# charlesq34/pointnet2

Measured on NVIDIA H100. Metric: set-abstraction points/sec, higher is better.
Workload: dtype f32

## Files before the change

include/pn2_api.h:

```cpp
#ifndef PN2_API_H_
#define PN2_API_H_

#include <stddef.h>

#ifdef __cplusplus
extern "C" {
#endif

#define PN2_API_VERSION 2


int pn2_fps(int b, int n, int m, const float* inp, float* temp, int* out, void* stream);

size_t pn2_fps_scratch_bytes(int b, int n);

int pn2_fps_gather(int b, int n, int m, const float* inp, float* temp, int* out, float* new_xyz, void* stream);


int pn2_fps_gather_ragged(int b, int n, int m, const float* inp, const int* lengths, float* temp, int* out,
                          float* new_xyz, void* stream);

int pn2_prob_sample(int b, int n, int m, const float* inp_p, const float* inp_r, float* temp, int* out, void* stream);

int pn2_gather_point(int b, int n, int m, const float* inp, const int* idx, float* out, void* stream);
// ... 184 lines not shown
size_t pn2_scene_blocks_workspace_bytes(int p, int nx, int ny);
int pn2_scene_blocks_count(int p, const float* xyz, double lo_x, double lo_y, double block_size, double stride, double padding,
                           int nx, int ny, int* counts, void* workspace, size_t workspace_bytes, void* stream);
int pn2_scene_blocks_fill(int p, const float* xyz, double lo_x, double lo_y, double block_size, double stride, double padding,
                          int nx, int ny, const int* sub_begin, const int* sub_count, int b, int n, float* out_xyz,
                          int* point_idx, unsigned char* core, int* occ_off, int* occ_row, void* workspace,
                          size_t workspace_bytes, void* stream);
int pn2_scene_merge_typed(int dtype, int p, int c, int b, int n, int row_begin, int row_end, const void* logits,
                          const int* point_idx, const unsigned char* core, const int* occ_off, const int* occ_row,
                          float* accum, void* stream);

size_t pn2_scene_crops_workspace_bytes(int b, int npoints);
int pn2_scene_crops(int s, int p, int max_scene, const float* xyz, const int* label, const long long* offsets, const float* lo,
                    const float* hi, int num_class, const float* label_weights, int b, const long long* crop_scene,
                    long long seed, const long long* seed_dev, int npoints, double max_dropout, int rotate, float* out_xyz,
                    long long* out_label, float* out_weight, int* lengths, int* point_idx, unsigned char* core, int* attempt,
                    unsigned char* valid, void* workspace, size_t workspace_bytes, void* stream);

int pn2_shape_batch(int s, int p, int max_shape, const float* xyz, const float* normals, const int* label, const int* part,
                    const long long* offsets, int b, const long long* shape_idx, long long seed, const long long* seed_dev,
                    int votes, int npoints, int subset_random, int rotate, int perturb, int scale_on, double scale_lo,
                    double scale_hi, double shift, int jitter_on, double jitter_sigma, double jitter_clip,
                    double max_dropout, int with_normals, float* out_points, long long* out_label, long long* out_part,
                    int* lengths, int* point_idx, void* stream);

size_t pn2_virtual_scans_workspace_bytes(int b, int max_scene, int npoints);
int pn2_virtual_scans(int s, int p, int max_scene, const float* xyz, const int* label, const long long* offsets,
                      const double* mean, int num_class, const float* label_weights, int b, const long long* scan_scene,
                      const long long* scan_mode, long long seed, const long long* seed_dev, int npoints, int min_points,
                      float* out_xyz, long long* out_label, float* out_weight, int* lengths, int* point_idx, int* visible,
                      unsigned char* valid, void* workspace, size_t workspace_bytes, void* stream);

size_t pn2_render_balls_workspace_bytes(int b, int h, int w);
int pn2_render_balls(int b, int n, int h, int w, const int* xyz, const float* colors, const int* lengths, int r,
                     const unsigned char* background, void* workspace, size_t workspace_bytes, unsigned char* out,
                     void* stream);
int pn2_render_balls_counted(int b, int n, int h, int w, const int* xyz, const float* colors, const int* lengths, int r,
                             const unsigned char* background, void* workspace, size_t workspace_bytes,
                             unsigned char* out, unsigned long long* counters, void* stream);
int pn2_project_points(int b, int n, int v, const double* xyz, const int* lengths, const double* rotations, int size,
                       void* workspace, size_t workspace_bytes, int* out, void* stream);


size_t pn2_sa_layer_workspace_bytes(int b, int n, int m, int nsample);
int pn2_sa_layer_host(int b, int n, int m, float radius, int nsample, const float* h_xyz,
                      float* h_new_xyz, int* h_idx, int* h_pts_cnt, float* h_grouped_xyz,
                      void* workspace, size_t workspace_bytes, void* stream);

int pn2_api_version(void);
const char* pn2_error_string(int code);
unsigned long long pn2_launch_count(void);
float pn2_ball_threshold(float radius);
void pn2_set_fps_config(int threads, int points_per_thread, int cluster);
int pn2_fps_plan(int b, int n, int* threads, int* points_per_thread, int* cluster);
int pn2_fps_cluster_capacity(int threads, int points_per_thread, int cluster);
void pn2_set_bq_group(int lanes_per_query);
void pn2_set_bq_mode(int mode);

#ifdef __cplusplus
}
#endif
#endif
```

pointnet2_b200/_lib.py:

```python
from __future__ import annotations

import ctypes
import os
from ctypes import c_double, c_float, c_int, c_longlong, c_size_t, c_ulonglong, c_void_p

from . import _build

_P = c_void_p
_SIGNATURES = {
    "pn2_fps": (c_int, [c_int, c_int, c_int, _P, _P, _P, _P]),
    "pn2_fps_scratch_bytes": (c_size_t, [c_int, c_int]),
    "pn2_fps_gather": (c_int, [c_int, c_int, c_int, _P, _P, _P, _P, _P]),
    "pn2_prob_sample": (c_int, [c_int, c_int, c_int, _P, _P, _P, _P, _P]),
    "pn2_gather_point": (c_int, [c_int, c_int, c_int, _P, _P, _P, _P]),
    "pn2_gather_point_grad": (c_int, [c_int, c_int, c_int, _P, _P, _P, _P]),
    "pn2_gather_point_grad_det": (c_int, [c_int, c_int, c_int, _P, _P, _P, _P, c_size_t, _P]),
    "pn2_query_ball_point": (c_int, [c_int, c_int, c_int, c_float, c_int, _P, _P, _P, _P, _P]),
    "pn2_query_ball_point_workspace_bytes": (c_size_t, [c_int, c_int]),
    "pn2_query_ball_point_ws": (c_int, [c_int, c_int, c_int, c_float, c_int, _P, _P, _P, _P, _P, c_size_t, _P]),
    "pn2_ball_grid_build": (c_int, [c_int, c_int, c_float, c_int, _P, _P, c_size_t, _P]),
    "pn2_query_ball_point_prebuilt": (c_int, [c_int, c_int, c_int, c_float, c_int, _P, _P, _P, _P, _P, c_size_t, _P]),
    "pn2_group_point": (c_int, [c_int, c_int, c_int, c_int, c_int, _P, _P, _P, _P]),
    "pn2_group_point_grad": (c_int, [c_int, c_int, c_int, c_int, c_int, _P, _P, _P, _P]),
    "pn2_group_point_grad_det_workspace_bytes": (c_size_t, [c_int, c_int, c_int, c_int]),
# ... 33 lines not shown
    "pn2_three_nn_ragged": (c_int, [c_int, c_int, c_int, _P, _P, _P, _P, _P, _P]),
    "pn2_three_nn_interpolate_ragged_typed": (c_int, [c_int, c_int, c_int, c_int, c_int, _P, _P, _P, _P, _P, _P, _P, _P, _P]),
    "pn2_fp_interpolate_concat_ragged_typed": (c_int, [c_int, c_int, c_int, c_int, c_int, c_int, _P, _P, _P, _P, _P, _P, _P]),
    "pn2_three_interpolate_ragged_typed": (c_int, [c_int, c_int, c_int, c_int, c_int, _P, _P, _P, _P, _P, _P]),
    "pn2_three_interpolate_grad_ragged": (c_int, [c_int, c_int, c_int, c_int, _P, _P, _P, _P, _P, _P]),
    "pn2_three_interpolate_grad_det_ragged_typed": (c_int, [c_int, c_int, c_int, c_int, c_int, _P, _P, _P, _P, _P, _P, c_size_t, _P]),
    "pn2_masked_bn_workspace_bytes": (c_size_t, [c_int, c_int]),
    "pn2_masked_bn_relu_forward_typed": (c_int, [c_int, c_int, c_int, _P, _P, _P, _P, c_float, c_float, _P, _P, _P, _P, _P, _P, _P,
                                                 c_size_t, _P]),
    "pn2_masked_bn_relu_backward_typed": (c_int, [c_int, c_int, c_int, _P, _P, _P, _P, _P, _P, _P, _P, _P, _P, _P, c_size_t, _P]),
    "pn2_masked_bn_relu_max_workspace_bytes": (c_size_t, [c_int, c_int, c_int]),
    "pn2_masked_bn_relu_max_forward_typed": (c_int, [c_int, c_int, c_int, c_int, _P, _P, _P, _P, c_float, c_float, _P, _P, _P,
                                                     _P, _P, _P, _P, _P, c_size_t, _P]),
    "pn2_masked_bn_relu_max_backward_typed": (c_int, [c_int, c_int, c_int, c_int, _P, _P, _P, _P, _P, _P, _P, _P, _P, _P, _P,
                                                      _P, c_size_t, _P]),
    "pn2_sa_mlp_max_typed": (c_int, [c_int, c_int, c_int, c_int, c_int, c_int, _P, _P, _P, _P, c_int, c_int, c_int, _P, _P, _P,
                                     _P, _P, _P, _P, _P, _P, _P, c_longlong, _P]),
    "pn2_sa_mlp_max_all_workspace_bytes": (c_size_t, [c_int, c_int]),
    "pn2_sa_mlp_max_all_typed": (c_int, [c_int, c_int, c_int, c_int, _P, _P, _P, _P, c_int, c_int, c_int, _P, _P, _P, _P, _P,
                                         _P, _P, _P, _P, _P, c_longlong, _P, c_size_t, _P]),
    "pn2_fp_mlp_workspace_bytes": (c_size_t, [c_int, c_int]),
    "pn2_fp_mlp_typed": (c_int, [c_int, c_int, c_int, c_int, c_int, c_int, _P, _P, _P, _P, _P, c_int, _P, _P, _P, _P, _P, _P,
                                 _P, _P, _P, _P, c_longlong, _P, c_size_t, _P]),
    "pn2_mlp_rows_typed": (c_int, [c_int, c_longlong, c_int, _P, _P, c_int, _P, _P, _P, _P, _P, _P, _P, _P, _P, _P, c_longlong,
                                   _P]),
    "pn2_scene_blocks_workspace_bytes": (c_size_t, [c_int, c_int, c_int]),
    "pn2_scene_blocks_count": (c_int, [c_int, _P, c_double, c_double, c_double, c_double, c_double, c_int, c_int, _P, _P,
                                       c_size_t, _P]),
    "pn2_scene_blocks_fill": (c_int, [c_int, _P, c_double, c_double, c_double, c_double, c_double, c_int, c_int, _P, _P,
                                      c_int, c_int, _P, _P, _P, _P, _P, _P, c_size_t, _P]),
    "pn2_scene_merge_typed": (c_int, [c_int, c_int, c_int, c_int, c_int, c_int, c_int, _P, _P, _P, _P, _P, _P, _P]),
    "pn2_scene_crops_workspace_bytes": (c_size_t, [c_int, c_int]),
    "pn2_scene_crops": (c_int, [c_int, c_int, c_int, _P, _P, _P, _P, _P, c_int, _P, c_int, _P, c_longlong, _P, c_int, c_double,
                                c_int, _P, _P, _P, _P, _P, _P, _P, _P, _P, c_size_t, _P]),
    "pn2_shape_batch": (c_int, [c_int, c_int, c_int, _P, _P, _P, _P, _P, c_int, _P, c_longlong, _P, c_int, c_int, c_int,
                                c_int, c_int, c_int, c_double, c_double, c_double, c_int, c_double, c_double, c_double,
                                c_int, _P, _P, _P, _P, _P, _P]),
    "pn2_virtual_scans_workspace_bytes": (c_size_t, [c_int, c_int, c_int]),
    "pn2_virtual_scans": (c_int, [c_int, c_int, c_int, _P, _P, _P, _P, c_int, _P, c_int, _P, _P, c_longlong, _P, c_int, c_int,
                                  _P, _P, _P, _P, _P, _P, _P, _P, c_size_t, _P]),
    "pn2_render_balls_workspace_bytes": (c_size_t, [c_int, c_int, c_int]),
    "pn2_render_balls": (c_int, [c_int, c_int, c_int, c_int, _P, _P, _P, c_int, _P, _P, c_size_t, _P, _P]),
    "pn2_render_balls_counted": (c_int, [c_int, c_int, c_int, c_int, _P, _P, _P, c_int, _P, _P, c_size_t, _P, _P, _P]),
    "pn2_project_points": (c_int, [c_int, c_int, c_int, _P, _P, _P, c_int, _P, c_size_t, _P, _P]),
    "pn2_sa_layer_workspace_bytes": (c_size_t, [c_int, c_int, c_int, c_int]),
    "pn2_sa_layer_host": (c_int, [c_int, c_int, c_int, c_float, c_int, _P, _P, _P, _P, _P, _P, c_size_t, _P]),
    "pn2_api_version": (c_int, []),
    "pn2_error_string": (ctypes.c_char_p, [c_int]),
    "pn2_launch_count": (c_ulonglong, []),
    "pn2_ball_threshold": (c_float, [c_float]),
    "pn2_fps_plan": (c_int, [c_int, c_int, _P, _P, _P]),
    "pn2_fps_cluster_capacity": (c_int, [c_int, c_int, c_int]),
    "pn2_set_fps_config": (None, [c_int, c_int, c_int]),
    "pn2_set_bq_group": (None, [c_int]),
    "pn2_set_bq_mode": (None, [c_int]),
}

EXPORTED_SYMBOLS = tuple(_SIGNATURES)

_lib = None


def lib_path() -> str:
    return _build.LIB_PATH


def load() -> ctypes.CDLL:
    global _lib
    if _lib is not None:
        return _lib
    path = _build.LIB_PATH
    world = int(os.environ.get("WORLD_SIZE", "1") or "1")
    local_rank = int(os.environ.get("LOCAL_RANK", "0") or "0")
    if world > 1:
        want = _build.source_signature()
        stamp = path + ".stamp"
        if local_rank == 0:
            if _build.is_stale():
                try:
                    _build.build()
                except Exception as e:
                    if not os.path.exists(path):
                        raise ImportError(f"libpn2_b200.so is missing and could not be built: {e}") from e
                    want = "prebuilt"
            tmp = stamp + f".tmp{os.getpid()}"
            with open(tmp, "w") as f:
                f.write(want)
            os.replace(tmp, stamp)
        else:
            import time
            deadline = time.time() + 600
            while time.time() < deadline:
                try:
                    got = open(stamp).read()
                except OSError:
                    got = None
                if got in (want, "prebuilt") and os.path.exists(path):
                    break
                time.sleep(0.2)
            else:
                raise ImportError("libpn2_b200.so was not (re)built by local rank 0 within 10 minutes")
    elif _build.is_stale():
        try:
            _build.build()
        except Exception as e:
            if not os.path.exists(path):
# ... 26 lines not shown
```

pointnet2_b200/csrc/fps.cu:

```cuda
#include <stdio.h>
#include <stdlib.h>

#include <atomic>
#include <mutex>

#include "pn2_common.cuh"

namespace pn2 {

__device__ __forceinline__ unsigned tb_encode(unsigned k) { return ((k & 511u) << 23) | (k >> 9); }
__device__ __forceinline__ unsigned tb_decode(unsigned tb) { return ((tb & 0x7fffffu) << 9) | (tb >> 23); }

__device__ __forceinline__ unsigned smem_addr(const void* p) { return (unsigned)__cvta_generic_to_shared(p); }
__device__ __forceinline__ unsigned cluster_ctarank() {
    unsigned r;
    asm volatile("mov.u32 %0, %%cluster_ctarank;" : "=r"(r));
    return r;
}
__device__ __forceinline__ unsigned cluster_nctarank() {
    unsigned r;
    asm volatile("mov.u32 %0, %%cluster_nctarank;" : "=r"(r));
    return r;
}
__device__ __forceinline__ void cluster_sync_all() {
// ... 214 lines not shown
        Z[h] = f2_pack(c[0][2], c[1][2]);
    }
    const unsigned tp = (tid < n) ? tb_encode((unsigned)tid) : 0xffffffffu;

    float x1 = src[0], y1 = src[1], z1 = src[2];
    if (tid == 0) write_pick(out, oxyz, 0, 0, x1, y1, z1);
    if (tid < 64) (&s_keys[0][0])[tid] = make_uint2(0xffffffffu, 0u);
    __syncthreads();

#pragma unroll 2
    for (int it = 1; it < m; ++it) {
        pair_update(X, Y, Z, td, x1, y1, z1);
        float g[G];
#pragma unroll
        for (int a = 0; a < G; ++a) {
            float v = td[GS * a];
#pragma unroll
            for (int u = 1; u < GS; ++u) v = fmaxf(v, td[GS * a + u]);
            g[a] = v;
        }
        float mx = 0.0f;
#pragma unroll
        for (int a = 0; a < G; ++a) mx = fmaxf(mx, g[a]);
        float s[GS];
#pragma unroll
        for (int u = 0; u < GS; ++u) s[u] = td[GS * (G - 1) + u];
        unsigned cg = SO::tbj(GS * (G - 1));
#pragma unroll
        for (int a = G - 2; a >= 0; --a) {
            const bool q = (g[a] == mx);
#pragma unroll
            for (int u = 0; u + 1 < GS; ++u) s[u] = q ? td[GS * a + u] : s[u];
            cg = q ? SO::tbj(GS * a) : cg;
        }
        unsigned cu = SO::tbj(GS - 1);
#pragma unroll
        for (int u = GS - 2; u >= 0; --u) cu = (s[u] == mx) ? SO::tbj(u) : cu;
        unsigned hi = __float_as_uint(mx), lo = tp | cg | cu;
        warp_max_min_pair(hi, lo);
        const int buf = it & 1;
        s_keys[buf][warp] = make_uint2(lo, hi);
        __syncthreads();
        const uint2 e = s_keys[buf][lane];
        unsigned gh = e.y, gl = e.x;
        warp_max_min_pair(gh, gl);
        const int old = (int)tb_decode(gl);
        x1 = src[3 * old + 0];
        y1 = src[3 * old + 1];
        z1 = src[3 * old + 2];
        if (tid == 0) write_pick(out, oxyz, it, old, x1, y1, z1);
    }
}

template <int P, int T, int V = 0, bool L = false>
__global__ void __launch_bounds__(T, 1)
fps_cta_kernel(int n, int m, const float* __restrict__ xyz, int* __restrict__ idx_out,
               float* __restrict__ new_xyz, int sentinel, const int* __restrict__ lengths) {
    static_assert(T % 512 == 0 || 512 % T == 0, "T must divide or be a multiple of the reference's 512 slots");
    __shared__ uint2 s_keys[2][32];
    extern __shared__ __align__(16) float s_xyz[];

    const int tid = threadIdx.x, lane = tid & 31, warp = tid >> 5;
    const int cloud = blockIdx.x;
    const float* __restrict__ pts = xyz + (size_t)cloud * n * 3;
    int* __restrict__ out = idx_out + (size_t)cloud * m;
    float* __restrict__ oxyz = new_xyz ? new_xyz + (size_t)cloud * m * 3 : nullptr;
    const int nb = L ? cloud_length(lengths, cloud, n) : n;

    const int total = 3 * nb;
    const bool vec = (reinterpret_cast<size_t>(pts) & 15) == 0;
    const int nv = vec ? (total >> 2) : 0;
    const float4* __restrict__ p4 = reinterpret_cast<const float4*>(pts);
    float4* __restrict__ s4 = reinterpret_cast<float4*>(s_xyz);
    constexpr int LB = 12;
    float4 v[LB];
#pragma unroll
    for (int u = 0; u < LB; ++u) {
        const int e = u * T + tid;
        if (e < nv) v[u] = __ldg(p4 + e);
    }
    if (sentinel) {
        for (int e = tid; e < m; e += T) out[e] = -1;
        __threadfence();
    }
#pragma unroll
    for (int u = 0; u < LB; ++u) {
        const int e = u * T + tid;
        if (e < nv) s4[e] = v[u];
    }
    for (int base = LB * T; base < nv; base += LB * T) {
#pragma unroll
        for (int u = 0; u < LB; ++u) {
            const int e = base + u * T + tid;
            if (e < nv) v[u] = __ldg(p4 + e);
        }
#pragma unroll
        for (int u = 0; u < LB; ++u) {
            const int e = base + u * T + tid;
            if (e < nv) s4[e] = v[u];
        }
    }
#pragma unroll 8
    for (int e = (nv << 2) + tid; e < total; e += T) s_xyz[e] = pts[e];
    __syncthreads();
    if (sentinel) pdl_launch_dependents();
    const float* __restrict__ src = s_xyz;

    if constexpr (V == 1) {
        fps_chain_packed<P, T>(nb, m, src, out, oxyz, s_keys);
    } else {
        constexpr int NW = T / 32;
        float px[P], py[P], pz[P], td[P];
#pragma unroll
        for (int j = 0; j < P; ++j) {
            const int k = tid + j * T;
            if (k < nb) {
                px[j] = src[3 * k + 0];
                py[j] = src[3 * k + 1];
                pz[j] = src[3 * k + 2];
                td[j] = 1e38f;
            } else {
                px[j] = py[j] = pz[j] = 0.0f;
                td[j] = -1.0f;
            }
        }

        float x1 = src[0], y1 = src[1], z1 = src[2];
        if (tid == 0) write_pick(out, oxyz, 0, 0, x1, y1, z1);

        for (int it = 1; it < m; ++it) {
            float best;
            int bj;
            fps_step<P, ScanOrder<P, T>::DD>(px, py, pz, td, x1, y1, z1, best, bj);
            unsigned hi = 0u, lo = 0u;
            if (best >= 0.0f) {
                hi = __float_as_uint(best);
                lo = ~tb_encode((unsigned)(tid + bj * T));
            }
            warp_max_pair(hi, lo);
            const int buf = it & 1;
            if (lane == 0) s_keys[buf][warp] = make_uint2(lo, hi);
            __syncthreads();
            uint2 e = (lane < NW) ? s_keys[buf][lane] : make_uint2(0u, 0u);
            unsigned gh = e.y, gl = e.x;
            warp_max_pair(gh, gl);
            const int old = (int)tb_decode(~gl);
            x1 = src[3 * old + 0];
            y1 = src[3 * old + 1];
            z1 = src[3 * old + 2];
            if (tid == 0) write_pick(out, oxyz, it, old, x1, y1, z1);
        }
    }
}

__device__ __forceinline__ void init_step_mbars(unsigned long long (&s_mbar)[2]) {
    mbar_init(smem_addr(&s_mbar[0]), 1);
    mbar_init(smem_addr(&s_mbar[1]), 1);
    fence_mbar_init_cluster();
}

template <int P, int PR, int T, class Keep>
// ... 368 lines not shown
                const float d2 = fminf(d, td[k]);
                td[k] = d2;
                if (d2 > best) {
                    best = d2;
                    bk = k;
                }
            }
            unsigned hi = 0u, lo = 0u;
            if (best >= 0.0f) {
                hi = __float_as_uint(best);
                lo = ~tb_encode((unsigned)bk);
            }
            warp_max_pair(hi, lo);
            const int buf = it & 1;
            if (lane == 0) s_keys[buf][warp] = make_uint2(lo, hi);
            __syncthreads();
            uint2 e = (lane < NW) ? s_keys[buf][lane] : make_uint2(0u, 0u);
            unsigned gh = e.y, gl = e.x;
            warp_max_pair(gh, gl);
            const int old = (int)tb_decode(~gl);
            x1 = pts[3 * (size_t)old + 0];
            y1 = pts[3 * (size_t)old + 1];
            z1 = pts[3 * (size_t)old + 2];
            if (tid == 0) {
                out[it] = old;
                if (oxyz) {
                    oxyz[3 * it + 0] = x1;
                    oxyz[3 * it + 1] = y1;
                    oxyz[3 * it + 2] = z1;
                }
            }
        }
        __syncthreads();
    }
}

static std::atomic<unsigned long long> g_fps_cfg{0ull};
static std::once_flag g_fps_env_once;
constexpr int kFpsPackedDefault = 1;
static std::atomic<int> g_fps_packed{kFpsPackedDefault};
constexpr int kFpsPackedClusterDefault = 1;
static std::atomic<int> g_fps_packed_cluster{kFpsPackedClusterDefault};

static int override_chain(int threads, int builtin) {
    const int chain = threads & 3;
    return chain == 1 ? 1 : (chain == 2 ? 0 : builtin);
}

static unsigned long long pack_cfg(int threads, int ppt, int cluster) {
    if (threads <= 0) return 0ull;
    return ((unsigned long long)threads << 40) | ((unsigned long long)(ppt & 0xfffff) << 20) | (unsigned long long)(cluster + 64);
}

template <int P, int T, int V>
static int launch_cta(int b, int n, int m, const float* inp, const int* lengths, int* out, float* new_xyz, int sentinel,
                      cudaStream_t st) {
    static AttrOnce once[2];
    auto kern = lengths ? fps_cta_kernel<P, T, V, true> : fps_cta_kernel<P, T, V, false>;
    size_t dyn = (size_t)n * 3 * sizeof(float);
    if (dyn > 200 * 1024) return (int)cudaErrorInvalidValue;
    constexpr size_t kExclusive = 116 * 1024;
    if (2 * b <= num_sms() && dyn < kExclusive) dyn = kExclusive;
    cudaError_t e = ensure_attrs(once[lengths ? 1 : 0], kern, 200 * 1024, false);
    if (e != cudaSuccess) return (int)e;
    kern<<<b, T, dyn, st>>>(n, m, inp, out, new_xyz, sentinel, lengths);
    return finish_launch();
}

static cudaLaunchConfig_t cluster_config(int clusters, int C, int T, size_t dyn, cudaStream_t st, cudaLaunchAttribute* attr) {
    cudaLaunchConfig_t cfg = {};
    cfg.gridDim = dim3((unsigned)clusters * (unsigned)C, 1, 1);
    cfg.blockDim = dim3(T, 1, 1);
    cfg.dynamicSmemBytes = dyn;
    cfg.stream = st;
    attr[0].id = cudaLaunchAttributeClusterDimension;
    attr[0].val.clusterDim.x = C;
    attr[0].val.clusterDim.y = 1;
    attr[0].val.clusterDim.z = 1;
    cfg.attrs = attr;
    cfg.numAttrs = 1;
    return cfg;
}

template <int P, int T, int PR, int V>
struct ClusterKernel {
    static constexpr size_t dyn = (size_t)3 * P * T * sizeof(float), max_dyn = 200 * 1024;
    static constexpr int threads = T;
    static auto kernel(bool ragged = false) { return ragged ? fps_cluster_kernel<P, T, PR, V, true> : fps_cluster_kernel<P, T, PR, V, false>; }
};
template <int P, int T, int PR, int V>
struct ClusterBigKernel {
    static constexpr size_t dyn = (size_t)3 * (P - PR) * T * sizeof(float), max_dyn = 226 * 1024;
    static constexpr int threads = T;
    static auto kernel(bool ragged = false) {
        return ragged ? fps_cluster_big_kernel<P, T, PR, V, true> : fps_cluster_big_kernel<P, T, PR, V, false>;
    }
};

template <class K>
static int launch_cluster(int C, int cluster_arg, int b, int n, int m, const float* inp, const int* lengths, int* out,
                          float* new_xyz, cudaStream_t st) {
    static AttrOnce once[2];
    if (K::dyn > K::max_dyn) return (int)cudaErrorInvalidValue;
    const bool ragged = lengths != nullptr;
    cudaError_t e = ensure_attrs(once[ragged ? 1 : 0], K::kernel(ragged), K::dyn, true);
    if (e != cudaSuccess) return (int)e;
    cudaLaunchAttribute attr[1];
    const cudaLaunchConfig_t cfg = cluster_config(b, C, K::threads, K::dyn, st, attr);
    e = cudaLaunchKernelEx(&cfg, K::kernel(ragged), n, m, cluster_arg, inp, out, new_xyz, lengths);
    count_launch();
    if (e != cudaSuccess) return (int)e;
    return (int)cudaGetLastError();
}

template <class K>
static int cluster_capacity(int C) {
    static std::atomic<int> cache[17][64];
    int dev = 0;
    if (C < 2 || C > 16 || cudaGetDevice(&dev) != cudaSuccess || dev < 0 || dev >= 64) return 0;
    const int hit = cache[C][dev].load(std::memory_order_relaxed);
    if (hit) return hit > 0 ? hit : 0;
    static AttrOnce once;
    if (K::dyn > K::max_dyn || ensure_attrs(once, K::kernel(), K::dyn, true) != cudaSuccess) return 0;
    cudaLaunchAttribute attr[1];
    const cudaLaunchConfig_t cfg = cluster_config(num_sms(), C, K::threads, K::dyn, nullptr, attr);
    int num = 0;
    if (cudaOccupancyMaxActiveClusters(&num, K::kernel(), &cfg) != cudaSuccess) {
        (void)cudaGetLastError();
        num = 0;
    }
    cache[C][dev].store(num > 0 ? num : -1, std::memory_order_relaxed);
    return num;
}

#define PN2_FPS_CTA_KERNELS(X)                                                                       \
    X(1, 128, 0) X(2, 128, 0) X(4, 128, 0) X(8, 128, 1) X(16, 128, 1) X(32, 128, 1)                  \
    X(1, 256, 0) X(2, 256, 0) X(4, 256, 0) X(8, 256, 1) X(16, 256, 1) X(32, 256, 1)                  \
    X(1, 512, 0) X(2, 512, 0) X(4, 512, 0) X(8, 512, 1) X(16, 512, 1)                                \
    X(1, 1024, 0) X(2, 1024, 0) X(4, 1024, 0) X(8, 1024, 1)
#define PN2_FPS_CLUSTER_KERNELS(X)                                                                   \
    X(4, 128, 4, 1) X(8, 128, 8, 1) X(16, 128, 16, 1) X(32, 128, 32, 1)                              \
    X(2, 256, 2, 0) X(4, 256, 4, 1) X(8, 256, 8, 1) X(16, 256, 16, 1) X(32, 256, 32, 1)              \
    X(1, 512, 1, 0) X(2, 512, 2, 0) X(4, 512, 4, 1) X(8, 512, 8, 1) X(16, 512, 16, 1) X(32, 512, 16, 1) \
    X(2, 1024, 2, 0) X(4, 1024, 4, 1) X(8, 1024, 8, 1)
#define PN2_FPS_BIG_KERNELS(X) X(44, 16) X(48, 12) X(52, 16)

struct FpsPlan {
    int threads, ppt, cluster;
    int pr;
    int packed = 0;
};

static int pow2_floor(int v) {
    int p = 1;
    while (p * 2 <= v) p *= 2;
    return p;
}

int fps_cluster_capacity(int threads, int ppt, int cluster, int packed);

static FpsPlan plan_fps(int b, int n) {
    std::call_once(g_fps_env_once, [] {
        const char* e = getenv("PN2_FPS_CFG");
        int t = 0, pp = 0, c = 0;
        if (e && sscanf(e, "%d,%d,%d", &t, &pp, &c) == 3) g_fps_cfg.store(pack_cfg(t, pp, c), std::memory_order_relaxed);
        const char* pk = getenv("PN2_FPS_PACKED");
        if (pk && (pk[0] == '0' || pk[0] == '1') && pk[1] == 0) g_fps_packed.store(pk[0] - '0', std::memory_order_relaxed);
        const char* pc = getenv("PN2_FPS_PACKED_CLUSTER");
        if (pc && (pc[0] == '0' || pc[0] == '1') && pc[1] == 0) g_fps_packed_cluster.store(pc[0] - '0', std::memory_order_relaxed);
    });
    const int packed = g_fps_packed.load(std::memory_order_relaxed);
    const int packed_cluster = g_fps_packed_cluster.load(std::memory_order_relaxed);
    const unsigned long long ov = g_fps_cfg.load(std::memory_order_relaxed);
    if (ov) {
        FpsPlan p;
        p.threads = (int)(ov >> 40);
        p.ppt = (int)((ov >> 20) & 0xfffff);
        p.cluster = (int)(ov & 0xfffff) - 64;
        p.packed = override_chain(p.threads, (p.cluster >= 2) ? packed_cluster : packed);
        p.threads &= ~3;
        p.pr = (p.ppt >= 32 && p.threads >= 512) ? 16 : p.ppt;
        if (p.cluster == -1 || p.cluster == -2) {
            p.packed = (p.cluster == -2) ? 1 : 0;
            p.cluster = 1;
        }
        return p;
    }
    if (n <= 128) return {128, 1, 1, 1, packed};
    if (n <= 256) return {128, 2, 1, 2, packed};
    if (n <= 512) return {256, 2, 1, 2, packed};
    if (n <= 1024) return {128, 8, 1, 8, packed};
    if (n <= 2048) return {128, 16, 1, 16, packed};
    if (n <= 4096) return {256, 16, 1, 16, packed};
    if (n <= 8192) return {256, 32, 1, 32, packed};
    const int sms = num_sms();
    int cmax = pow2_floor(sms / (b > sms ? sms : b));
    if (cmax > 16) cmax = 16;
    if (cmax < 2) cmax = 2;
    auto pick = [packed_cluster](long long per, int C, FpsPlan& out) -> bool {
        const int t = (C >= 4) ? 128 : 256;
        const int pmin = (t == 128) ? 4 : 2;
        for (int pp = pmin; pp <= 32; pp *= 2) {
            if (per <= (long long)t * pp) {
                out = {t, pp, C, pp, packed_cluster};
                return true;
            }
        }
        if (per <= 256LL * 32) {
            out = {256, 32, C, 32, packed_cluster};
            return true;
        }
        if (per <= 512LL * 32) {
            out = {512, 32, C, 16, packed_cluster};
            return true;
        }
        return false;
    };
    FpsPlan first{0, 0, 0, 0};
    for (int C = cmax; C >= 2; C /= 2) {
        const long long per = ((long long)n + C - 1) / C;
        if (per <= 1024 && C > 2) continue;
        FpsPlan p;
        if (!pick(per, C, p)) break;
        if (first.cluster == 0) first = p;
        const int cap = fps_cluster_capacity(p.threads, p.ppt, p.cluster, p.packed);
        if (cap == 0 || cap >= b) return p;
    }
    FpsPlan best{0, 0, 0, 0};
    double best_cost = 1e30;
    auto consider = [&](const FpsPlan& p) {
        const int cap = fps_cluster_capacity(p.threads, p.ppt, p.cluster, p.packed);
        const int waves = cap > 0 ? (b + cap - 1) / cap : 1;
        double cost = waves * (0.3 + 0.07e-3 * (double)p.threads * p.ppt);
        if (cap > 0 && (long long)cap * p.cluster > sms) cost *= 1.3;
        if (cost < best_cost) {
            best_cost = cost;
            best = p;
        }
    };
    if (first.cluster) consider(first);
    FpsPlan widest;
    if (pick(((long long)n + 15) / 16, 16, widest)) consider(widest);
    for (int C = 16; C >= 2; --C) {
        const long long per = ((long long)n + C - 1) / C;
        if (per > 512LL * 52) break;
        consider({512, per <= 512LL * 44 ? 44 : (per <= 512LL * 48 ? 48 : 52), C, 16, packed_cluster});
    }
    if (best.cluster) return best;
    return {1024, 0, 0, 0};
}

bool fps_single_cta(int b, int n) { return plan_fps(b, n).cluster == 1; }

size_t fps_scratch_bytes(int b, int n) {
    if (b <= 0 || n <= 0) return 0;
    return plan_fps(b, n).cluster == 0 ? sizeof(float) * (size_t)(b < 32 ? b : 32) * (size_t)n : 0;
}

int fps_dispatch(int b, int n, int m, const float* inp, const int* lengths, float* temp, int* out, float* new_xyz,
                 int sentinel, cudaStream_t st) {
    if (b < 0 || n <= 0 || m < 0) return (int)cudaErrorInvalidValue;
    if (b == 0 || m == 0) return 0;
    if (!inp || !out) return (int)cudaErrorInvalidValue;
    const FpsPlan plan = plan_fps(b, n);
    if (sentinel && plan.cluster != 1) return (int)cudaErrorInvalidValue;
    if (plan.cluster >= 1) {
        const long long cap = (long long)plan.threads * plan.ppt * plan.cluster;
        if (cap < n) return (int)cudaErrorInvalidValue;
    }
    if (plan.cluster == 1) {
#define PN2_TRY(P, T, PK)                                                                           \
    if (plan.ppt == P && plan.threads == T)                                                                 \
        return (PK && plan.packed) ? launch_cta<P, T, PK>(b, n, m, inp, lengths, out, new_xyz, sentinel, st)         \
                                   : launch_cta<P, T, 0>(b, n, m, inp, lengths, out, new_xyz, sentinel, st);
        PN2_FPS_CTA_KERNELS(PN2_TRY)
#undef PN2_TRY
        return (int)cudaErrorInvalidValue;
    }
    const int C = plan.cluster;
    if (C >= 2 && plan.ppt > 32) {
        if (C > 16 || plan.threads != 512) return (int)cudaErrorInvalidValue;
#define PN2_TRY(P, PR)                                                                                       \
    if (plan.ppt == P)                                                                                               \
        return plan.packed ? launch_cluster<ClusterBigKernel<P, 512, PR, 1>>(C, C, b, n, m, inp, lengths, out, new_xyz, st)  \
                           : launch_cluster<ClusterBigKernel<P, 512, PR, 0>>(C, C, b, n, m, inp, lengths, out, new_xyz, st);
        PN2_FPS_BIG_KERNELS(PN2_TRY)
#undef PN2_TRY
        return (int)cudaErrorInvalidValue;
    }
    if (C >= 2) {
        if (C > 16 || (C & (C - 1))) return (int)cudaErrorInvalidValue;
        if (((long long)C * plan.threads) % 512 != 0) return (int)cudaErrorInvalidValue;
        int log2c = 0;
        while ((1 << log2c) < C) ++log2c;
#define PN2_TRY(P, T, PR, PK)                                                                                 \
    if (plan.ppt == P && plan.threads == T && plan.pr == PR)                                                  \
        return (PK && plan.packed)                                                                            \
                   ? launch_cluster<ClusterKernel<P, T, PR, PK>>(C, log2c, b, n, m, inp, lengths, out, new_xyz, st)    \
                   : launch_cluster<ClusterKernel<P, T, PR, 0>>(C, log2c, b, n, m, inp, lengths, out, new_xyz, st);
        PN2_FPS_CLUSTER_KERNELS(PN2_TRY)
#undef PN2_TRY
        return (int)cudaErrorInvalidValue;
    }
    if (!temp) return (int)cudaErrorInvalidValue;
    int grid = b < 32 ? b : 32;
    fps_global_kernel<1024><<<grid, 1024, 0, st>>>(b, n, m, inp, temp, out, new_xyz, lengths);
    return finish_launch();
}

int fps_cluster_capacity(int threads, int ppt, int cluster, int packed) {
#define PN2_CAP(P, PR)                                                                                      \
    if (threads == 512 && ppt == P)                                                                         \
        return packed ? cluster_capacity<ClusterBigKernel<P, 512, PR, 1>>(cluster)                          \
                      : cluster_capacity<ClusterBigKernel<P, 512, PR, 0>>(cluster);
    PN2_FPS_BIG_KERNELS(PN2_CAP)
#undef PN2_CAP
    if (cluster < 2 || cluster > 16 || (cluster & (cluster - 1))) return 0;
#define PN2_CAP(P, T, PR, PK)                                                                               \
    if (ppt == P && threads == T)                                                                           \
        return (PK && packed) ? cluster_capacity<ClusterKernel<P, T, PR, PK>>(cluster)                      \
                              : cluster_capacity<ClusterKernel<P, T, PR, 0>>(cluster);
    PN2_FPS_CLUSTER_KERNELS(PN2_CAP)
#undef PN2_CAP
    return 0;
}

}

extern "C" {

int pn2_fps_cluster_capacity(int threads, int points_per_thread, int cluster) {
    const int packed = pn2::override_chain(threads, pn2::g_fps_packed_cluster.load(std::memory_order_relaxed));
    return pn2::fps_cluster_capacity(threads & ~3, points_per_thread, cluster, packed);
}

int pn2_fps(int b, int n, int m, const float* inp, float* temp, int* out, void* stream) {
    return pn2::fps_dispatch(b, n, m, inp, nullptr, temp, out, nullptr, 0, pn2::as_stream(stream));
}

int pn2_fps_gather(int b, int n, int m, const float* inp, float* temp, int* out, float* new_xyz, void* stream) {
    return pn2::fps_dispatch(b, n, m, inp, nullptr, temp, out, new_xyz, 0, pn2::as_stream(stream));
}

int pn2_fps_gather_ragged(int b, int n, int m, const float* inp, const int* lengths, float* temp, int* out, float* new_xyz,
                          void* stream) {
    return pn2::fps_dispatch(b, n, m, inp, lengths, temp, out, new_xyz, 0, pn2::as_stream(stream));
}

size_t pn2_fps_scratch_bytes(int b, int n) { return pn2::fps_scratch_bytes(b, n); }

int pn2_fps_plan(int b, int n, int* threads, int* points_per_thread, int* cluster) {
    if (b <= 0 || n <= 0) return (int)cudaErrorInvalidValue;
    const pn2::FpsPlan p = pn2::plan_fps(b, n);
    if (threads) *threads = p.threads;
    if (points_per_thread) *points_per_thread = p.ppt;
    if (cluster) *cluster = p.cluster;
    return 0;
}

void pn2_set_fps_config(int threads, int points_per_thread, int cluster) {
    pn2::g_fps_cfg.store(pn2::pack_cfg(threads, points_per_thread, cluster), std::memory_order_relaxed);
}

}
```

Measured before the change: 379.0 million.

## Add spatially sorted FPS chain that skips warps via bounding-box distance bounds

Adds a new FPS variant that Morton-sorts points in shared memory with a two-pass radix sort, so each warp owns a spatially compact set of points. Each warp keeps a bounding box and skips the distance update and argmax whenever the box lower bound cannot beat its current max distance. It becomes the default for the 4097-8192 point CTA plan. The cost is a sort prologue, extra shared memory and a divergent branch. A counting entry point is also added to measure how many warps are reached per iteration.

```diff
diff --git a/include/pn2_api.h b/include/pn2_api.h
--- a/include/pn2_api.h
+++ b/include/pn2_api.h
@@ -260,6 +260,7 @@
 unsigned long long pn2_launch_count(void);
 float pn2_ball_threshold(float radius);
 void pn2_set_fps_config(int threads, int points_per_thread, int cluster);
+int pn2_fps_cull_counts(int b, int n, int m, const float* inp, int* out, unsigned* counts, void* stream);
 int pn2_fps_plan(int b, int n, int* threads, int* points_per_thread, int* cluster);
 int pn2_fps_cluster_capacity(int threads, int points_per_thread, int cluster);
 void pn2_set_bq_group(int lanes_per_query);
diff --git a/pointnet2_b200/_lib.py b/pointnet2_b200/_lib.py
--- a/pointnet2_b200/_lib.py
+++ b/pointnet2_b200/_lib.py
@@ -109,6 +109,7 @@
     "pn2_fps_plan": (c_int, [c_int, c_int, _P, _P, _P]),
     "pn2_fps_cluster_capacity": (c_int, [c_int, c_int, c_int]),
     "pn2_set_fps_config": (None, [c_int, c_int, c_int]),
+    "pn2_fps_cull_counts": (c_int, [c_int, c_int, c_int, _P, _P, _P, _P]),
     "pn2_set_bq_group": (None, [c_int]),
     "pn2_set_bq_mode": (None, [c_int]),
 }
diff --git a/pointnet2_b200/csrc/fps.cu b/pointnet2_b200/csrc/fps.cu
--- a/pointnet2_b200/csrc/fps.cu
+++ b/pointnet2_b200/csrc/fps.cu
@@ -290,10 +290,277 @@
     }
 }
 
-template <int P, int T, int V = 0, bool L = false>
+__device__ __forceinline__ unsigned morton_spread4(unsigned v) {
+    return (v & 1u) | ((v & 2u) << 2) | ((v & 4u) << 4) | ((v & 8u) << 6);
+}
+__device__ __forceinline__ unsigned morton_cell(float v, float lo, float s) {
+    const int q = __float2int_rz(__fmul_rn(__fsub_rn(v, lo), s));
+    return (unsigned)min(max(q, 0), 15);
+}
+
+template <int T>
+__device__ __forceinline__ int cta_exclusive_scan(int v, int* s_w) {
+    const int lane = threadIdx.x & 31, warp = threadIdx.x >> 5;
+    int incl = v;
+#pragma unroll
+    for (int o = 1; o < 32; o <<= 1) {
+        const int t = __shfl_up_sync(kFullMask, incl, o);
+        if (lane >= o) incl += t;
+    }
+    if (lane == 31) s_w[warp] = incl;
+    __syncthreads();
+    int off = 0;
+#pragma unroll
+    for (int w = 0; w < T / 32; ++w) off += (w < warp) ? s_w[w] : 0;
+    __syncthreads();
+    return off + incl - v;
+}
+
+__device__ __forceinline__ unsigned same_digit_lanes(unsigned d, unsigned active) {
+    unsigned mask = active;
+#pragma unroll
+    for (int bit = 0; bit < 6; ++bit) {
+        const unsigned b = __ballot_sync(kFullMask, (d >> bit) & 1u);
+        mask &= ((d >> bit) & 1u) ? b : ~b;
+    }
+    return mask;
+}
+
+template <int T>
+__device__ void cull_radix_pass(int nb, const unsigned short* in, unsigned short* out, const unsigned short* s_code,
+                                int shift, int* s_tab, int* s_w) {
+    constexpr int NW = T / 32;
+    const int tid = threadIdx.x, lane = tid & 31, warp = tid >> 5;
+    s_tab[2 * tid] = 0;
+    s_tab[2 * tid + 1] = 0;
+    __syncthreads();
+    const int per = (nb + NW - 1) / NW;
+    const int k0 = warp * per, k1 = min(nb, k0 + per);
+    const unsigned lt = (1u << lane) - 1u;
+    for (int p = k0 + lane; p < k1; p += 32) {
+        const unsigned k = in ? in[p] : (unsigned)p;
+        atomicAdd(&s_tab[(((unsigned)s_code[k] >> shift) & 63u) * NW + warp], 1);
+    }
+    __syncthreads();
+    const int a = s_tab[2 * tid], b = s_tab[2 * tid + 1];
+    const int ex = cta_exclusive_scan<T>(a + b, s_w);
+    s_tab[2 * tid] = ex;
+    s_tab[2 * tid + 1] = ex + a;
+    __syncthreads();
+    for (int base = k0; base < k1; base += 32) {
+        const int p = base + lane;
+        const bool valid = p < k1;
+        const unsigned k = valid ? (in ? in[p] : (unsigned)p) : 0u;
+        const unsigned d = ((unsigned)s_code[k] >> shift) & 63u;
+        const unsigned mask = same_digit_lanes(d, __ballot_sync(kFullMask, valid));
+        const int first = valid ? s_tab[d * NW + warp] : 0;
+        if (valid) out[first + __popc(mask & lt)] = (unsigned short)k;
+        __syncwarp();
+        if (valid && (mask & lt) == 0) s_tab[d * NW + warp] = first + __popc(mask);
+        __syncwarp();
+    }
+    __syncthreads();
+}
+
+template <int P>
+__device__ __forceinline__ void sort_words(unsigned (&w)[P]) {
+#pragma unroll
+    for (int k = 2; k <= P; k <<= 1) {
+#pragma unroll
+        for (int j = k >> 1; j > 0; j >>= 1) {
+#pragma unroll
+            for (int i = 0; i < P; ++i) {
+                const int l = i ^ j;
+                if (l > i) {
+                    const unsigned a = w[i], b = w[l];
+                    const bool up = (i & k) == 0;
+                    w[i] = up ? min(a, b) : max(a, b);
+                    w[l] = up ? max(a, b) : min(a, b);
+                }
+            }
+        }
+    }
+}
+
+template <int P>
+__device__ __forceinline__ void value_argmax_word(const float (&td)[P], const unsigned (&tb)[P], float& mx, unsigned& word) {
+    static_assert(P % 4 == 0, "groups of four");
+    constexpr int G = P / 4;
+    float g[G];
+#pragma unroll
+    for (int a = 0; a < G; ++a) g[a] = fmaxf(fmaxf(fmaxf(td[4 * a], td[4 * a + 1]), td[4 * a + 2]), td[4 * a + 3]);
+    float m = 0.0f;
+#pragma unroll
+    for (int a = 0; a < G; ++a) m = fmaxf(m, g[a]);
+    float s0 = td[4 * (G - 1)], s1 = td[4 * (G - 1) + 1], s2 = td[4 * (G - 1) + 2];
+    unsigned w0 = tb[4 * (G - 1)], w1 = tb[4 * (G - 1) + 1], w2 = tb[4 * (G - 1) + 2], w3 = tb[4 * (G - 1) + 3];
+#pragma unroll
+    for (int a = G - 2; a >= 0; --a) {
+        const bool q = (g[a] == m);
+        s0 = q ? td[4 * a] : s0;
+        s1 = q ? td[4 * a + 1] : s1;
+        s2 = q ? td[4 * a + 2] : s2;
+        w0 = q ? tb[4 * a] : w0;
+        w1 = q ? tb[4 * a + 1] : w1;
+        w2 = q ? tb[4 * a + 2] : w2;
+        w3 = q ? tb[4 * a + 3] : w3;
+    }
+    unsigned w = w3;
+    w = (s2 == m) ? w2 : w;
+    w = (s1 == m) ? w1 : w;
+    w = (s0 == m) ? w0 : w;
+    mx = m;
+    word = w;
+}
+
+template <int P, int T, bool CNT>
+__device__ __forceinline__ void fps_chain_culled(int nb, int m, const float* __restrict__ src, int* __restrict__ out,
+                                                 float* __restrict__ oxyz, uint2 (&s_keys)[2][32],
+                                                 unsigned short* __restrict__ s_sort, unsigned* __restrict__ counts) {
+    constexpr int NW = T / 32, NK = T * P, H = P / 2;
+    static_assert(P % 4 == 0 && NK <= 8192, "groups of four; point indices fit the 16-bit sort entries");
+    __shared__ float s_box[32][6];
+    __shared__ int s_w[32];
+    __shared__ int s_tab[2 * T];
+    const int tid = threadIdx.x, lane = tid & 31, warp = tid >> 5;
+
+    float lx = INFINITY, ly = INFINITY, lz = INFINITY, hx = -INFINITY, hy = -INFINITY, hz = -INFINITY;
+    int bad = 0;
+    for (int k = tid; k < nb; k += T) {
+        const float x = src[3 * k + 0], y = src[3 * k + 1], z = src[3 * k + 2];
+        bad |= !(isfinite(x) && isfinite(y) && isfinite(z));
+        lx = fminf(lx, x);
+        ly = fminf(ly, y);
+        lz = fminf(lz, z);
+        hx = fmaxf(hx, x);
+        hy = fmaxf(hy, y);
+        hz = fmaxf(hz, z);
+    }
+    lx = warp_min_f32(lx);
+    ly = warp_min_f32(ly);
+    lz = warp_min_f32(lz);
+    hx = warp_max_f32(hx);
+    hy = warp_max_f32(hy);
+    hz = warp_max_f32(hz);
+    if (lane == 0) {
+        s_box[warp][0] = lx;
+        s_box[warp][1] = ly;
+        s_box[warp][2] = lz;
+        s_box[warp][3] = hx;
+        s_box[warp][4] = hy;
+        s_box[warp][5] = hz;
+    }
+    const bool all = __syncthreads_or(bad) != 0;
+#pragma unroll
+    for (int w = 0; w < NW; ++w) {
+        lx = fminf(lx, s_box[w][0]);
+        ly = fminf(ly, s_box[w][1]);
+        lz = fminf(lz, s_box[w][2]);
+        hx = fmaxf(hx, s_box[w][3]);
+        hy = fmaxf(hy, s_box[w][4]);
+        hz = fmaxf(hz, s_box[w][5]);
+    }
+    auto cells_per_unit = [](float lo, float hi) {
+        const float e = __fsub_rn(hi, lo);
+        return e > 0.0f ? __fdiv_rn(16.0f, e) : 0.0f;
+    };
+    const float sx = cells_per_unit(lx, hx), sy = cells_per_unit(ly, hy), sz = cells_per_unit(lz, hz);
+
+    unsigned short *s_code = s_sort, *s_a = s_sort + NK, *s_b = s_sort + 2 * NK;
+    for (int k = tid; k < nb; k += T) {
+        s_code[k] = (unsigned short)(morton_spread4(morton_cell(src[3 * k + 0], lx, sx)) |
+                                     (morton_spread4(morton_cell(src[3 * k + 1], ly, sy)) << 1) |
+                                     (morton_spread4(morton_cell(src[3 * k + 2], lz, sz)) << 2));
+    }
+    __syncthreads();
+    cull_radix_pass<T>(nb, nullptr, s_a, s_code, 0, s_tab, s_w);
+    cull_radix_pass<T>(nb, s_a, s_b, s_code, 6, s_tab, s_w);
+
+    unsigned tb[P];
+#pragma unroll
+    for (int e = 0; e < P; ++e) {
+        const int p = tid * P + e;
+        tb[e] = (p < nb) ? tb_encode(s_b[p]) : 0xffffffffu;
+    }
+    sort_words<P>(tb);
+    unsigned long long X[H], Y[H], Z[H];
+    float td[P];
+    float bx0 = INFINITY, by0 = INFINITY, bz0 = INFINITY, bx1 = -INFINITY, by1 = -INFINITY, bz1 = -INFINITY;
+#pragma unroll
+    for (int h = 0; h < H; ++h) {
+        float c[2][3];
+#pragma unroll
+        for (int u = 0; u < 2; ++u) {
+            const int e = 2 * h + u;
+            c[u][0] = c[u][1] = c[u][2] = 0.0f;
+            td[e] = -1.0f;
+            if (tb[e] != 0xffffffffu) {
+                const int k = (int)tb_decode(tb[e]);
+                c[u][0] = src[3 * k + 0];
+                c[u][1] = src[3 * k + 1];
+                c[u][2] = src[3 * k + 2];
+                td[e] = 1e38f;
+                bx0 = fminf(bx0, c[u][0]);
+                by0 = fminf(by0, c[u][1]);
+                bz0 = fminf(bz0, c[u][2]);
+                bx1 = fmaxf(bx1, c[u][0]);
+                by1 = fmaxf(by1, c[u][1]);
+                bz1 = fmaxf(bz1, c[u][2]);
+            }
+        }
+        X[h] = f2_pack(c[0][0], c[1][0]);
+        Y[h] = f2_pack(c[0][1], c[1][1]);
+        Z[h] = f2_pack(c[0][2], c[1][2]);
+    }
+    float mx = (tb[0] != 0xffffffffu) ? 1e38f : 0.0f;
+    unsigned wh = __float_as_uint(mx), wl = tb[0];
+    warp_max_min_pair(wh, wl);
+
+    float x1 = src[0], y1 = src[1], z1 = src[2];
+    if (tid == 0) write_pick(out, oxyz, 0, 0, x1, y1, z1);
+    if (tid < 64) (&s_keys[0][0])[tid] = make_uint2(0xffffffffu, 0u);
+    __syncthreads();
+
+#pragma unroll 2
+    for (int it = 1; it < m; ++it) {
+        const float gx = fmaxf(fmaxf(__fsub_rn(bx0, x1), __fsub_rn(x1, bx1)), 0.0f);
+        const float gy = fmaxf(fmaxf(__fsub_rn(by0, y1), __fsub_rn(y1, by1)), 0.0f);
+        const float gz = fmaxf(fmaxf(__fsub_rn(bz0, z1), __fsub_rn(z1, bz1)), 0.0f);
+        const float lb = __fmaf_rn(gz, gz, __fmaf_rn(gx, gx, __fmul_rn(gy, gy)));
+        const unsigned reached = __ballot_sync(kFullMask, all || lb < mx);
+        if constexpr (CNT) {
+            if (lane == 0 && reached) {
+                atomicAdd(&counts[2 * it], (unsigned)__popc(reached));
+                atomicAdd(&counts[2 * it + 1], 1u);
+            }
+        }
+        if (reached) {
+            pair_update(X, Y, Z, td, x1, y1, z1);
+            unsigned lo;
+            value_argmax_word<P>(td, tb, mx, lo);
+            unsigned hi = __float_as_uint(mx);
+            warp_max_min_pair(hi, lo);
+            wh = hi;
+            wl = lo;
+        }
+        const int buf = it & 1;
+        s_keys[buf][warp] = make_uint2(wl, wh);
+        __syncthreads();
+        const uint2 e = s_keys[buf][lane];
+        unsigned gh = e.y, gl = e.x;
+        warp_max_min_pair(gh, gl);
+        const int old = (int)tb_decode(gl);
+        x1 = src[3 * old + 0];
+        y1 = src[3 * old + 1];
+        z1 = src[3 * old + 2];
+        if (tid == 0) write_pick(out, oxyz, it, old, x1, y1, z1);
+    }
+}
+
+template <int P, int T, int V = 0, bool L = false, bool CNT = false>
 __global__ void __launch_bounds__(T, 1)
 fps_cta_kernel(int n, int m, const float* __restrict__ xyz, int* __restrict__ idx_out,
-               float* __restrict__ new_xyz, int sentinel, const int* __restrict__ lengths) {
+               float* __restrict__ new_xyz, int sentinel, const int* __restrict__ lengths, unsigned* __restrict__ counts) {
     static_assert(T % 512 == 0 || 512 % T == 0, "T must divide or be a multiple of the reference's 512 slots");
     __shared__ uint2 s_keys[2][32];
     extern __shared__ __align__(16) float s_xyz[];
@@ -344,7 +611,9 @@
     if (sentinel) pdl_launch_dependents();
     const float* __restrict__ src = s_xyz;
 
-    if constexpr (V == 1) {
+    if constexpr (V == 2) {
+        fps_chain_culled<P, T, CNT>(nb, m, src, out, oxyz, s_keys, reinterpret_cast<unsigned short*>(s_xyz + 3 * n), counts);
+    } else if constexpr (V == 1) {
         fps_chain_packed<P, T>(nb, m, src, out, oxyz, s_keys);
     } else {
         constexpr int NW = T / 32;
@@ -819,18 +1088,18 @@
     return ((unsigned long long)threads << 40) | ((unsigned long long)(ppt & 0xfffff) << 20) | (unsigned long long)(cluster + 64);
 }
 
-template <int P, int T, int V>
+template <int P, int T, int V, bool CNT = false>
 static int launch_cta(int b, int n, int m, const float* inp, const int* lengths, int* out, float* new_xyz, int sentinel,
-                      cudaStream_t st) {
+                      cudaStream_t st, unsigned* counts = nullptr) {
     static AttrOnce once[2];
-    auto kern = lengths ? fps_cta_kernel<P, T, V, true> : fps_cta_kernel<P, T, V, false>;
-    size_t dyn = (size_t)n * 3 * sizeof(float);
+    auto kern = lengths ? fps_cta_kernel<P, T, V, true, CNT> : fps_cta_kernel<P, T, V, false, CNT>;
+    size_t dyn = (size_t)n * 3 * sizeof(float) + (V == 2 ? (size_t)3 * T * P * sizeof(unsigned short) : 0);
     if (dyn > 200 * 1024) return (int)cudaErrorInvalidValue;
     constexpr size_t kExclusive = 116 * 1024;
     if (2 * b <= num_sms() && dyn < kExclusive) dyn = kExclusive;
     cudaError_t e = ensure_attrs(once[lengths ? 1 : 0], kern, 200 * 1024, false);
     if (e != cudaSuccess) return (int)e;
-    kern<<<b, T, dyn, st>>>(n, m, inp, out, new_xyz, sentinel, lengths);
+    kern<<<b, T, dyn, st>>>(n, m, inp, out, new_xyz, sentinel, lengths, counts);
     return finish_launch();
 }
 
@@ -900,11 +1169,11 @@
     return num;
 }
 
-#define PN2_FPS_CTA_KERNELS(X)                                                                       \
-    X(1, 128, 0) X(2, 128, 0) X(4, 128, 0) X(8, 128, 1) X(16, 128, 1) X(32, 128, 1)                  \
-    X(1, 256, 0) X(2, 256, 0) X(4, 256, 0) X(8, 256, 1) X(16, 256, 1) X(32, 256, 1)                  \
-    X(1, 512, 0) X(2, 512, 0) X(4, 512, 0) X(8, 512, 1) X(16, 512, 1)                                \
-    X(1, 1024, 0) X(2, 1024, 0) X(4, 1024, 0) X(8, 1024, 1)
+#define PN2_FPS_CTA_KERNELS(X)                                                                            \
+    X(1, 128, 0, 0) X(2, 128, 0, 0) X(4, 128, 0, 0) X(8, 128, 1, 1) X(16, 128, 1, 1) X(32, 128, 1, 0)     \
+    X(1, 256, 0, 0) X(2, 256, 0, 0) X(4, 256, 0, 0) X(8, 256, 1, 0) X(16, 256, 1, 1) X(32, 256, 1, 1)     \
+    X(1, 512, 0, 0) X(2, 512, 0, 0) X(4, 512, 0, 0) X(8, 512, 1, 1) X(16, 512, 1, 0)                      \
+    X(1, 1024, 0, 0) X(2, 1024, 0, 0) X(4, 1024, 0, 0) X(8, 1024, 1, 0)
 #define PN2_FPS_CLUSTER_KERNELS(X)                                                                   \
     X(4, 128, 4, 1) X(8, 128, 8, 1) X(16, 128, 16, 1) X(32, 128, 32, 1)                              \
     X(2, 256, 2, 0) X(4, 256, 4, 1) X(8, 256, 8, 1) X(16, 256, 16, 1) X(32, 256, 32, 1)              \
@@ -947,8 +1216,8 @@
         p.packed = override_chain(p.threads, (p.cluster >= 2) ? packed_cluster : packed);
         p.threads &= ~3;
         p.pr = (p.ppt >= 32 && p.threads >= 512) ? 16 : p.ppt;
-        if (p.cluster == -1 || p.cluster == -2) {
-            p.packed = (p.cluster == -2) ? 1 : 0;
+        if (p.cluster == -1 || p.cluster == -2 || p.cluster == -3) {
+            p.packed = -p.cluster - 1;
             p.cluster = 1;
         }
         return p;
@@ -959,7 +1228,7 @@
     if (n <= 1024) return {128, 8, 1, 8, packed};
     if (n <= 2048) return {128, 16, 1, 16, packed};
     if (n <= 4096) return {256, 16, 1, 16, packed};
-    if (n <= 8192) return {256, 32, 1, 32, packed};
+    if (n <= 8192) return {256, 32, 1, 32, packed == kFpsPackedDefault ? 2 : packed};
     const int sms = num_sms();
     int cmax = pow2_floor(sms / (b > sms ? sms : b));
     if (cmax > 16) cmax = 16;
@@ -1036,10 +1305,14 @@
         if (cap < n) return (int)cudaErrorInvalidValue;
     }
     if (plan.cluster == 1) {
-#define PN2_TRY(P, T, PK)                                                                           \
-    if (plan.ppt == P && plan.threads == T)                                                                 \
-        return (PK && plan.packed) ? launch_cta<P, T, PK>(b, n, m, inp, lengths, out, new_xyz, sentinel, st)         \
-                                   : launch_cta<P, T, 0>(b, n, m, inp, lengths, out, new_xyz, sentinel, st);
+#define PN2_TRY(P, T, PK, CU)                                                                                  \
+    if (plan.ppt == P && plan.threads == T) {                                                                  \
+        if (plan.packed == 2)                                                                                  \
+            return CU ? launch_cta<P, T, CU ? 2 : 0>(b, n, m, inp, lengths, out, new_xyz, sentinel, st)        \
+                      : (int)cudaErrorInvalidValue;                                                            \
+        return (PK && plan.packed) ? launch_cta<P, T, PK>(b, n, m, inp, lengths, out, new_xyz, sentinel, st)   \
+                                   : launch_cta<P, T, 0>(b, n, m, inp, lengths, out, new_xyz, sentinel, st);   \
+    }
         PN2_FPS_CTA_KERNELS(PN2_TRY)
 #undef PN2_TRY
         return (int)cudaErrorInvalidValue;
@@ -1073,6 +1346,20 @@
     int grid = b < 32 ? b : 32;
     fps_global_kernel<1024><<<grid, 1024, 0, st>>>(b, n, m, inp, temp, out, new_xyz, lengths);
     return finish_launch();
+}
+
+int fps_cull_counts(int b, int n, int m, const float* inp, int* out, unsigned* counts, cudaStream_t st) {
+    if (b <= 0 || n <= 0 || m <= 0 || !inp || !out || !counts) return (int)cudaErrorInvalidValue;
+    const FpsPlan plan = plan_fps(b, n);
+    if (plan.cluster != 1 || (long long)plan.threads * plan.ppt < n) return (int)cudaErrorInvalidValue;
+    cudaError_t e = cudaMemsetAsync(counts, 0, sizeof(unsigned) * 2 * (size_t)m, st);
+    if (e != cudaSuccess) return (int)e;
+#define PN2_TRY(P, T, PK, CU)                                                                              \
+    if (CU && plan.ppt == P && plan.threads == T)                                                          \
+        return launch_cta<P, T, CU ? 2 : 0, CU != 0>(b, n, m, inp, nullptr, out, nullptr, 0, st, counts);
+    PN2_FPS_CTA_KERNELS(PN2_TRY)
+#undef PN2_TRY
+    return (int)cudaErrorInvalidValue;
 }
 
 int fps_cluster_capacity(int threads, int ppt, int cluster, int packed) {
@@ -1116,6 +1403,10 @@
 
 size_t pn2_fps_scratch_bytes(int b, int n) { return pn2::fps_scratch_bytes(b, n); }
 
+int pn2_fps_cull_counts(int b, int n, int m, const float* inp, int* out, unsigned* counts, void* stream) {
+    return pn2::fps_cull_counts(b, n, m, inp, out, counts, pn2::as_stream(stream));
+}
+
 int pn2_fps_plan(int b, int n, int* threads, int* points_per_thread, int* cluster) {
     if (b <= 0 || n <= 0) return (int)cudaErrorInvalidValue;
     const pn2::FpsPlan p = pn2::plan_fps(b, n);
```

After: 379.1 million (median of 6 runs). No clear change (+0.0%).
